# albertz/ParseOggVorbis

Measured on AMD Instinct MI355X. Metric: audio packets/sec (blocksize 2048, stereo), higher is better.
Workload: dtype f32; 1 GPU; config3: 65536 stereo packets, blocksize 2048, 64 streams x 1024, floor+coupling+IMDCT+window+overlap-add; packets_per_gpu=65536, parallelism=streams sharded over 1 GPU(s), no data-path collective

## Files before the change

parseoggvorbis_amd/csrc/vorbis_synth_hip.hip:

```cpp
#include <hip/hip_runtime.h>

#include <mutex>
#include <string>

#include <stdlib.h>

#include "vsyn_host.h"
#include "vsyn_device.h"
#include "vsyn_staged.h"
#include "vsyn_prep.h"
#include "vsyn_fused.h"
#include "vsyn_fused_u.h"
#include "vsyn_vq.h"
#include "vsyn_pcm.h"
#include "vsyn_features.h"
#include "vsyn_spectral.h"
#include "vsyn_spectral_lin.h"
#include "vsyn_spectral_post.h"
#include "vsyn_resample.h"
#include "vsyn_condition.h"
#include "vsyn_trim.h"
#include "vsyn_split.h"
#include "vsyn_pitch.h"
#include "vsyn_fdesc.h"
// ... 349 lines not shown
      fail(err, VSYN_ERR_HIP, "generic fused table upload failed: %s", hipGetErrorString(e));
      return cleanup(VSYN_ERR_HIP);
    }
  }
#undef HC
  *out = h;
  return VSYN_OK;
}

void vsyn_destroy(vsyn_handle* h) {
  if (!h) return;
  (void)hipSetDevice(h->device);
  (void)hipDeviceSynchronize();
  vq_stamps_dump();
  prep_stamps_dump();
  fused_stamps_dump();
  fused_tables_destroy(&h->fused);
  u_tables_destroy(&h->utab);
  if (h->side) (void)hipStreamDestroy(h->side);
  if (h->pre) (void)hipStreamDestroy(h->pre);
  if (h->host_stream) (void)hipStreamDestroy(h->host_stream);
  if (h->ev_join) (void)hipEventDestroy(h->ev_join);
  if (h->ev_self) (void)hipEventDestroy(h->ev_self);
  if (h->ev_reset) (void)hipEventDestroy(h->ev_reset);
  for (uint32_t b = 0; b < vsyn_handle::WS_RING; ++b)
    if (h->ev_pre_done[b]) (void)hipEventDestroy(h->ev_pre_done[b]);
  for (uint32_t b = 0; b < vsyn_handle::EV_RING; ++b)
    if (h->ev_ring[b]) (void)hipEventDestroy(h->ev_ring[b]);
  if (h->d_const) (void)hipFree(h->d_const);
  if (h->d_vq) (void)hipFree(h->d_vq);
  if (h->d_state) (void)hipFree(h->d_state);
  if (h->d_carry) (void)hipFree(h->d_carry);
  if (h->d_status) (void)hipFree(h->d_status);
  for (auto& ev : h->events) {
    (void)hipEventDestroy(ev.first);
    (void)hipEventDestroy(ev.second);
  }
  delete h;
}

uint32_t vsyn_ys_stride(const vsyn_handle* h) { return h ? h->H.ys_stride : 0; }
uint32_t vsyn_channels(const vsyn_handle* h) { return h ? h->H.channels : 0; }
uint32_t vsyn_fused_paths(const vsyn_handle* h) { return h ? (h->fused_mask | (h->vq_tables_in_lds ? 0x100u : 0u)) : 0; }
size_t vsyn_const_block_bytes(const vsyn_handle* h) { return h ? h->host_const.size() : 0; }

int vsyn_profile_enable(vsyn_handle* h, int on) {
  if (!h) return VSYN_ERR_INVALID;
  h->profile = on != 0;
  if (on >= 1 && on <= 3) h->profile_which = on;
  return VSYN_OK;
}

int vsyn_profile_read(vsyn_handle* h, double* mean_ms, uint32_t* launches, const char** kernel_name) {
  if (!h) return VSYN_ERR_INVALID;
  std::lock_guard<std::mutex> lk(h->mu);
  (void)hipSetDevice(h->device);
  double total = 0;
  for (size_t i = 0; i < h->events_used; ++i) {
    (void)hipEventSynchronize(h->events[i].second);
    float ms = 0;
    (void)hipEventElapsedTime(&ms, h->events[i].first, h->events[i].second);
    total += ms;
  }
  if (mean_ms) *mean_ms = h->events_used ? total / (double)h->events_used : 0.0;
  if (launches) *launches = (uint32_t)h->events_used;
  if (kernel_name) *kernel_name = h->profile_kernel;
  h->events_used = 0;
  return VSYN_OK;
}

static hipError_t profile_begin(vsyn_handle* h, hipStream_t s, const char* name) {
  if (!h->profile) return hipSuccess;
  if (h->events_used == h->events.size()) {
    hipEvent_t a, b;
    const unsigned pf = hipEventDisableSystemFence;
    hipError_t e = hipEventCreateWithFlags(&a, pf);
    if (e != hipSuccess) return e;
    e = hipEventCreateWithFlags(&b, pf);
    if (e != hipSuccess) return e;
    h->events.emplace_back(a, b);
  }
  h->profile_kernel = name;
  return hipEventRecord(h->events[h->events_used].first, s);
}
static hipError_t profile_end(vsyn_handle* h, hipStream_t s) {
  if (!h->profile) return hipSuccess;
  hipError_t e = hipEventRecord(h->events[h->events_used].second, s);
  ++h->events_used;
  return e;
}

int vsyn_reset_streams(vsyn_handle* h, void* hip_stream, const char** err) {
  if (!h) return fail(err, VSYN_ERR_INVALID, "handle is NULL");
  std::lock_guard<std::mutex> lk(h->mu);
  HIPCHK(hipSetDevice(h->device));
  HIPCHK(hipMemsetAsync(h->d_state, 0, sizeof(StreamState) * 2 * h->H.max_streams, (hipStream_t)hip_stream));
  HIPCHK(hipEventRecord(h->ev_reset, (hipStream_t)hip_stream));
  h->reset_pending = true;
  return VSYN_OK;
}

int vsyn_sync_status(vsyn_handle* h, void* hip_stream, vsyn_status* status, const char** err) {
  if (!h) return fail(err, VSYN_ERR_INVALID, "handle is NULL");
  HIPCHK(hipSetDevice(h->device));
  HIPCHK(hipStreamSynchronize((hipStream_t)hip_stream));
  DevStatus ds;
  HIPCHK(hipMemcpy(&ds, h->d_status, sizeof(ds), hipMemcpyDeviceToHost));
  if (ds.flags) {
    DevStatus init = {0u, 0xFFFFFFFFu};
    HIPCHK(hipMemcpy(h->d_status, &init, sizeof(init), hipMemcpyHostToDevice));
  }
  if (status) {
    status->flags = ds.flags;
    status->first_bad_packet = ds.first_bad_packet;
  }
  if (ds.flags) return fail(err, VSYN_ERR_STREAM, "device flagged the batch: flags=0x%x first_bad_packet=%u", ds.flags, ds.first_bad_packet);
  return VSYN_OK;
}

static int submit_device_impl(vsyn_handle* h, uint32_t P, const vsyn_packet* d_packets, uint32_t S, const vsyn_segment* d_segments,
                              uint32_t max_seg_packets, const uint16_t* d_ys, const vsyn_vq_batch* d_vq, float* d_residue, float* d_pcm,
                              uint64_t plane_stride, uint32_t* d_emit_len, const vsyn_taps* taps, uint32_t flags, void* hip_stream,
                              const char** err) {
  if (!h) return fail(err, VSYN_ERR_INVALID, "handle is NULL");
  if (P == 0 || S == 0) return VSYN_OK;
  if (!d_packets || !d_segments || !d_ys || !d_residue || !d_pcm) return fail(err, VSYN_ERR_INVALID, "NULL batch pointer");
  if (d_vq) {
    if (!h->d_vq) return fail(err, VSYN_ERR_INVALID, "vsyn_attach_vq has not been called on this handle");
    if (!d_vq->packets || (d_vq->num_cls && !d_vq->cls) || (d_vq->num_entries && !d_vq->entries)) return fail(err, VSYN_ERR_INVALID, "NULL vq batch pointer");
  }
  if (max_seg_packets == 0 || max_seg_packets > P) max_seg_packets = P;
  std::lock_guard<std::mutex> lk(h->mu);
  HIPCHK(hipSetDevice(h->device));
  hipStream_t s = (hipStream_t)hip_stream;
  const ConstHeader& H = h->H;
  const uint32_t C = H.channels;

  const bool want_taps = taps && (taps->after_envelope || taps->pcm_after_mdct);
  const bool use_u = h->u_mixed;
  const uint32_t fmask = h->fused_mask;
  const bool force_staged = want_taps || (flags & VSYN_SUBMIT_STAGED) || !fmask;
  const uint32_t R = force_staged ? std::min<uint32_t>(max_seg_packets, 1024u)
                                  : fused_pick_run_len(h->opt.run_len, (fmask & 1u) || !use_u ? h->fused.waves_per_cu : (int)h->utab.waves_per_cu,
                                                       S, C, max_seg_packets, h->num_cus);
  const uint32_t runs_per_seg = (max_seg_packets + R - 1) / R;

  const bool prep_kernel = !force_staged && (fmask & 2u) && !d_vq && max_seg_packets <= PREP_MAX_SEG_PACKETS && !(flags & VSYN_SUBMIT_PRE_KERNELS);
  hipStream_t ps = !prep_kernel && (flags & VSYN_SUBMIT_INPUTS_READY) && !force_staged ? h->pre : s;
  const uint32_t chunk_packets = max_seg_packets <= LAYOUT_CHUNK_PACKETS ? runs_per_seg * R : (LAYOUT_CHUNK_PACKETS + R - 1u) / R * R;
  const uint32_t chunks_per_seg = (max_seg_packets + chunk_packets - 1u) / chunk_packets;
  const uint32_t prep_nt = std::min<uint32_t>(PREP_THREADS, std::max<uint32_t>(64u, ((max_seg_packets * C + 63u) / 64u) * 64u));
  const uint32_t prep_chunk_runs = std::max<uint32_t>(1u, std::max<uint32_t>(1u, prep_nt / C) / R);
  const uint32_t prep_chunks_per_seg = (runs_per_seg + prep_chunk_runs - 1u) / prep_chunk_runs;
  const uint64_t prep_wgs = (((uint64_t)S * prep_chunks_per_seg + 7u) / 8u) * 16u;
  const bool staged_may_work = force_staged || !(fmask & 2u);
  hipStream_t ss = force_staged ? s : h->side;
  const uint64_t fused_units = (uint64_t)S * runs_per_seg * C;

  if (!prep_kernel && (uint64_t)S * chunks_per_seg > 0x7FFFFFFFull) return fail(err, VSYN_ERR_INVALID, "too many layout chunks");
  if (prep_kernel && prep_wgs > 0x7FFFFFF0ull) return fail(err, VSYN_ERR_INVALID, "too many runs");
  if (!force_staged && fused_units > (use_u ? U_MAX_UNITS : FUSED_MAX_UNITS)) return fail(err, VSYN_ERR_INVALID, "too many runs");
  const uint64_t isub = h->nsub;
  const uint32_t wb = (uint32_t)(isub % vsyn_handle::WS_RING), wb_prev = (uint32_t)((isub + vsyn_handle::WS_RING - 1u) % vsyn_handle::WS_RING);
  HIPCHK(h->ws_info[wb].ensure((size_t)P + 8));
  HIPCHK(h->ws_seg[wb].ensure(S));
  HIPCHK(h->ws_segmap[wb].ensure(P));
  HIPCHK(h->ws_list[wb].ensure(2 * (size_t)P + 64));
  uint16_t* fy = taps && taps->floor_final ? taps->floor_final : nullptr;
  if (!fy) {
    HIPCHK(h->ws_fy[wb].ensure((size_t)P * C * H.ys_stride));
    fy = h->ws_fy[wb].p;
  }
  HIPCHK(h->ws_runcls[wb].ensure((size_t)S * runs_per_seg + 16));
  bool clear_chunks = false;
  if (!prep_kernel && chunks_per_seg > 1 && (size_t)S * chunks_per_seg > h->ws_chunks.cap) {
    HIPCHK(h->ws_chunks.ensure((size_t)S * chunks_per_seg));
    clear_chunks = true;
  }
  float* env = taps && taps->after_envelope ? taps->after_envelope : nullptr;
  float* blk = taps && taps->pcm_after_mdct ? taps->pcm_after_mdct : nullptr;
  if (staged_may_work) {
    const size_t bound = (size_t)P * C * (H.bs[1] / 2);
    if (!env) {
      HIPCHK(h->ws_env.ensure(bound));
      env = h->ws_env.p;
    }
    if (!blk) {
      HIPCHK(h->ws_blk.ensure(2 * bound));
      blk = h->ws_blk.p;
    }
  }
  PktInfo* info = h->ws_info[wb].p;
  SegInfo* sinfo = h->ws_seg[wb].p;
  uint32_t* segmap = h->ws_segmap[wb].p;
  uint32_t* list = h->ws_list[wb].p;

  ++h->nsub;
  uint32_t* cnt = h->ws_count.p + (isub % vsyn_handle::CNT_RING);
  uint32_t* cnt_next = h->ws_count.p + ((isub + 1u) % vsyn_handle::CNT_RING);
  ++h->submit_count;
  const uint32_t epoch = (h->submit_count & 0x3FFFFFFFu) ? h->submit_count : ++h->submit_count;
  if (ps != s) {
    if (isub >= vsyn_handle::WS_RING) {
      const uint64_t need = isub - vsyn_handle::WS_RING;
      const uint32_t slot = (uint32_t)(need % vsyn_handle::EV_RING);
      if (h->ev_ring_submit[slot] == need) {
        HIPCHK(hipStreamWaitEvent(ps, h->ev_ring[slot], 0));
      } else {
        HIPCHK(hipEventRecord(h->ev_self, s));
        HIPCHK(hipStreamWaitEvent(ps, h->ev_self, 0));
      }
    }
    if (h->last_prep_on_main && isub > 0) {
      HIPCHK(hipEventRecord(h->ev_self, s));
      HIPCHK(hipStreamWaitEvent(ps, h->ev_self, 0));
    }
  }
  if (h->pre_done_valid[wb_prev] && h->last_pre_stream != ps) HIPCHK(hipStreamWaitEvent(ps, h->ev_pre_done[wb_prev], 0));
  if (h->reset_pending) HIPCHK(hipStreamWaitEvent(ps, h->ev_reset, 0));

  if (!prep_kernel) {
    if (!h->last_ran_layout) HIPCHK(hipMemsetAsync(h->ws_count.p, 0, sizeof(uint32_t) * vsyn_handle::CNT_RING, ps));
    if (clear_chunks) HIPCHK(hipMemsetAsync(h->ws_chunks.p, 0, h->ws_chunks.cap * sizeof(LayoutChunk), ps));
    const uint32_t lt = std::min(chunk_packets, max_seg_packets) <= LAYOUT_SHORT_PACKETS ? LAYOUT_THREADS_SHORT : LAYOUT_THREADS;
    vsyn_layout_kernel<<<S * chunks_per_seg, lt, layout_lds_bytes(lt, chunk_packets), ps>>>(
        h->d_const, P, d_packets, S, d_segments, plane_stride, info, sinfo, h->d_state, d_emit_len, h->d_status, R, force_staged ? 0u : fmask, list, cnt,
        cnt_next, segmap, h->ws_runcls[wb].p, runs_per_seg, chunk_packets, chunks_per_seg, h->ws_chunks.p, epoch);
    const uint32_t rows = P * C;
    vsyn_floor_unwrap_kernel<<<(rows + UNWRAP_THREADS - 1) / UNWRAP_THREADS, UNWRAP_THREADS, h->unwrap_lds_bytes, ps>>>(h->d_const, P, info, d_ys, fy,
                                                                                                                          h->d_status);
    if (d_vq) {
      if (h->profile_which == 3) HIPCHK(profile_begin(h, ps, "vsyn_residue_vq_kernel"));
      if (h->vq_tables_in_lds)
        vsyn_residue_vq_kernel<true><<<std::min<uint32_t>((P + h->vq_waves - 1u) / h->vq_waves, h->vq_grid), VQ_THREADS * h->vq_waves, h->vq_lds_bytes, ps>>>(
            h->d_const, h->d_vq, P, info, d_vq->packets, d_vq->cls, d_vq->num_cls, d_vq->entries, d_vq->num_entries, d_residue, h->d_status);
      else
        vsyn_residue_vq_kernel<false><<<std::min<uint32_t>(P, h->vq_grid), VQ_THREADS, h->vq_lds_bytes, ps>>>(
            h->d_const, h->d_vq, P, info, d_vq->packets, d_vq->cls, d_vq->num_cls, d_vq->entries, d_vq->num_entries, d_residue, h->d_status);
      if (h->profile_which == 3) HIPCHK(profile_end(h, ps));
    }
  } else {
    PrepCtx pc;
    pc.cb = h->d_const;
    pc.packets = d_packets;
    pc.segs = d_segments;
    pc.ys = d_ys;
    pc.fy = fy;
    pc.info = info;
    pc.sinfo = sinfo;
    pc.state = h->d_state;
    pc.status = h->d_status;
    pc.emit_len = d_emit_len;
    pc.run_cls = h->ws_runcls[wb].p;
    pc.plane_stride = plane_stride;
    pc.long_modes = h->long_modes;
    pc.S = S;
    pc.R = R;
    pc.runs_per_seg = runs_per_seg;
    pc.fused_ok = fmask;
    pc.P = P;
    pc.epoch = epoch;
    pc.chunk_runs = prep_chunk_runs;
    pc.chunks_per_seg = prep_chunks_per_seg;
    vsyn_prep_kernel<<<(uint32_t)prep_wgs, prep_nt, h->prep_lds_bytes, ps>>>(pc);
  }
  if (ps != s) {
    HIPCHK(hipEventRecord(h->ev_pre_done[wb], ps));
    HIPCHK(hipStreamWaitEvent(s, h->ev_pre_done[wb], 0));
  }

  if (staged_may_work) {
    if (!force_staged) {
      if (ps != s) {
        HIPCHK(hipStreamWaitEvent(h->side, h->ev_pre_done[wb], 0));
      } else {
        HIPCHK(hipEventRecord(h->ev_self, s));
        HIPCHK(hipStreamWaitEvent(h->side, h->ev_self, 0));
      }
    }
    const uint32_t grid = force_staged ? std::min<uint32_t>(P * C, 256u * 32u) : 512u;
    vsyn_spectrum_kernel<<<std::min<uint32_t>(grid, P), 256, 0, ss>>>(h->d_const, list, cnt, info, d_residue, fy, env,
                                                                      taps ? taps->floor_curve : nullptr, h->d_status);
    if (force_staged) HIPCHK(profile_begin(h, s, "vsyn_imdct_staged_kernel"));
    vsyn_imdct_staged_kernel<<<grid, 256, (size_t)H.bs[1] * 4, ss>>>(h->d_const, list, cnt, info, env, blk);
    if (force_staged) HIPCHK(profile_end(h, s));
    vsyn_overlap_kernel<<<grid, 256, 0, ss>>>(h->d_const, list, cnt, info, d_segments, sinfo, segmap, blk, d_pcm, plane_stride, h->d_carry);
  }
  if (!force_staged) {
    FusedArgs a;
    a.cb = h->d_const;
    a.binseg = h->fused.d_binseg;
    a.lds_image = h->fused.d_lds;
    a.packets = d_packets;
    a.segs = d_segments;
    a.info = info;
    a.sinfo = sinfo;
    a.run_cls = h->ws_runcls[wb].p;
    a.runs_per_seg = runs_per_seg;
    a.residue = d_residue;
    a.curve = taps ? taps->floor_curve : nullptr;
    a.fy = fy;
    a.pcm = d_pcm;
    a.carry = h->d_carry;
    a.status = h->d_status;
    a.plane_stride = plane_stride;
    a.S = S;
    a.R = R;
    a.fused_ok = use_u ? (fmask & 1u) : fmask;
    a.coupling_mode = (uint32_t)h->fused.coupling_mode;
    if (staged_may_work) HIPCHK(hipEventRecord(h->ev_join, h->side));
    const bool time_u = use_u && (h->profile_which == 2 || !(fmask & 1u));
    hipError_t e = hipSuccess;
    if (a.fused_ok) {
      if (!time_u && (h->profile_which == 1 || h->profile_which == 2)) HIPCHK(profile_begin(h, s, a.curve ? "vsyn_fused_tap_kernel" : fused_kernel_name(H)));
      e = fused_launch(H, h->fused, a, s);
      if (e != hipSuccess) return fail(err, VSYN_ERR_HIP, "fused launch failed: %s", hipGetErrorString(e));
      if (!time_u && (h->profile_which == 1 || h->profile_which == 2)) HIPCHK(profile_end(h, s));
    }
    if (use_u) {
      FusedArgs au = a;
      au.fused_ok = fmask;
      if (time_u && (h->profile_which == 1 || h->profile_which == 2)) HIPCHK(profile_begin(h, s, au.curve ? "vsyn_fused_u_tap_kernel" : "vsyn_fused_u_kernel"));
      e = u_launch(H, h->utab, au, s);
      if (e != hipSuccess) return fail(err, VSYN_ERR_HIP, "generic fused launch failed: %s", hipGetErrorString(e));
      if (time_u && (h->profile_which == 1 || h->profile_which == 2)) HIPCHK(profile_end(h, s));
    }
    if (staged_may_work) HIPCHK(hipStreamWaitEvent(s, h->ev_join, 0));
  }

  h->last_ran_layout = !prep_kernel;
  h->last_prep_on_main = ps == s;
  h->pre_done_valid[wb] = ps != s;
  h->last_pre_stream = ps;
  h->reset_pending = false;
  if (ps != s) {
    const uint32_t slot = (uint32_t)(isub % vsyn_handle::EV_RING);
    HIPCHK(hipEventRecord(h->ev_ring[slot], s));
    h->ev_ring_submit[slot] = isub;
  }
  h->last_S = S;
  h->last_wb = wb;
  HIPCHK(hipGetLastError());
  return VSYN_OK;
}

int vsyn_submit_device(vsyn_handle* h, uint32_t P, const vsyn_packet* d_packets, uint32_t S, const vsyn_segment* d_segments,
                       uint32_t max_seg_packets, const uint16_t* d_ys, const float* d_residue, float* d_pcm,
                       uint64_t plane_stride, uint32_t* d_emit_len, const vsyn_taps* taps, uint32_t flags, void* hip_stream,
                       const char** err) {
  return submit_device_impl(h, P, d_packets, S, d_segments, max_seg_packets, d_ys, nullptr, const_cast<float*>(d_residue), d_pcm, plane_stride,
                            d_emit_len, taps, flags, hip_stream, err);
}

int vsyn_submit_device_vq(vsyn_handle* h, uint32_t P, const vsyn_packet* d_packets, uint32_t S, const vsyn_segment* d_segments,
                          uint32_t max_seg_packets, const uint16_t* d_ys, const vsyn_vq_batch* d_vq, float* d_residue, float* d_pcm,
                          uint64_t plane_stride, uint32_t* d_emit_len, const vsyn_taps* taps, uint32_t flags, void* hip_stream,
                          const char** err) {
  if (!d_vq) return fail(err, VSYN_ERR_INVALID, "vq batch is NULL");
  return submit_device_impl(h, P, d_packets, S, d_segments, max_seg_packets, d_ys, d_vq, d_residue, d_pcm, plane_stride, d_emit_len, taps, flags,
                            hip_stream, err);
}

int vsyn_attach_vq(vsyn_handle* h, const vsyn_vq_setup* vq, const char** err) {
  if (!h) return fail(err, VSYN_ERR_INVALID, "handle is NULL");
  std::vector<uint8_t> block;
  const std::string why = vq_build_block(vq, h->H, block);
  if (!why.empty()) return fail(err, VSYN_ERR_INVALID, "%s", why.c_str());
  std::lock_guard<std::mutex> lk(h->mu);
  HIPCHK(hipSetDevice(h->device));
  const uint32_t lds_budget = 156u * 1024u;
  HIPCHK(hipFuncSetAttribute((const void*)vsyn_residue_vq_kernel<true>, hipFuncAttributeMaxDynamicSharedMemorySize, (int)lds_budget));
  HIPCHK(hipDeviceSynchronize());
  if (h->d_vq) (void)hipFree(h->d_vq);
  h->d_vq = nullptr;
  HIPCHK(hipMalloc((void**)&h->d_vq, block.size()));
  HIPCHK(hipMemcpy(h->d_vq, block.data(), block.size(), hipMemcpyHostToDevice));
  const VqHeader* vh = (const VqHeader*)block.data();
  uint32_t lds_off[7];
  const uint32_t wave_bytes = vq_lds_layout(vh->max_slots, vh->max_classes, lds_off);
  h->vq_tables_in_lds = false;
  h->vq_waves = 1;
  if (vh->img_floats && !h->opt.vq_no_lds_tables) {
    const uint32_t tab_bytes = vq_align16(vh->img_floats * 4u);
    hipFuncAttributes fa;
    HIPCHK(hipFuncGetAttributes(&fa, (const void*)vsyn_residue_vq_kernel<true>));
    const uint32_t regs = ((uint32_t)std::max(fa.numRegs, 1) + 7u) / 8u * 8u;
    const uint32_t cu_waves = 4u * std::min<uint32_t>(8u, 512u / regs);
    uint32_t best_k = 0, best_w = 0;
    for (uint32_t k = 1; k <= 4; ++k) {
      const uint32_t budget = k == 1 ? lds_budget : 128u * 1024u;
      if (budget / k <= tab_bytes + wave_bytes) break;
      const uint32_t w = std::min<uint32_t>({16u, (budget / k - tab_bytes) / wave_bytes, cu_waves / k});
      if (w && k * w > best_k * best_w) best_k = k, best_w = w;
    }
    if (best_w) {
      const uint32_t lds = tab_bytes + best_w * wave_bytes;
      int per_cu = 0;
      HIPCHK(hipOccupancyMaxActiveBlocksPerMultiprocessor(&per_cu, vsyn_residue_vq_kernel<true>, (int)(VQ_THREADS * best_w), lds));
      if (per_cu > 0) {
        h->vq_tables_in_lds = true;
        h->vq_waves = best_w;
        h->vq_lds_bytes = lds;
        h->vq_grid = (uint32_t)h->num_cus * (uint32_t)per_cu;
        if (h->opt.debug) fprintf(stderr, "[vsyn] vq: tables in LDS (%u B), %u waves per workgroup, %d workgroups per CU, %u B LDS\n", tab_bytes, best_w, per_cu, lds);
      }
    }
  }
  if (!h->vq_tables_in_lds) {
    h->vq_lds_bytes = wave_bytes;
    int per_cu = 0;
    HIPCHK(hipOccupancyMaxActiveBlocksPerMultiprocessor(&per_cu, vsyn_residue_vq_kernel<false>, VQ_THREADS, h->vq_lds_bytes));
    h->vq_grid = (uint32_t)h->num_cus * (uint32_t)std::max(per_cu, 1);
  }
  return VSYN_OK;
}

// ... 1105 lines not shown
```

parseoggvorbis_amd/csrc/vsyn_prep.h:

```cpp
#pragma once
#include <hip/hip_runtime.h>

#include "vsyn_device.h"
#include "vsyn_floor1.h"
#include "vsyn_staged.h"

#define PREP_MAX_SEG_PACKETS 4096u
#define PREP_WAVES 4
#define PREP_THREADS (PREP_WAVES * 64)

struct PrepCtx {
  const uint8_t* cb;
  const vsyn_packet* packets;
  const vsyn_segment* segs;
  const uint16_t* ys;
  uint16_t* fy;
  PktInfo* info;
  SegInfo* sinfo;
  StreamState* state;
  DevStatus* status;
  uint32_t* emit_len;
  uint8_t* run_cls;
  uint64_t plane_stride, long_modes;
  uint32_t S, R, runs_per_seg, fused_ok, P, epoch;
  uint32_t chunk_runs, chunks_per_seg;
};

#ifdef PREP_STAMPS
#define PREP_NSTAMPS 8
__device__ unsigned long long g_prep_stamps[8192][PREP_NSTAMPS];
#define PSTAMP(i)                                                \
  do {                                                           \
    __builtin_amdgcn_sched_barrier(0);                           \
    const unsigned long long t_ = __builtin_readcyclecounter();  \
    pst_acc[i] += t_ - pst_last;                                 \
    pst_last = t_;                                               \
    __builtin_amdgcn_sched_barrier(0);                           \
  } while (0)
#else
#define PSTAMP(i) do { } while (0)
#endif

__device__ __forceinline__ void prep_wave_scan(AbsScan& inc, uint64_t& rinc, const uint32_t lane) {
#pragma unroll
  for (int d = 1; d < 64; d <<= 1) {
    const AbsScan o = abs_shfl_up(inc, d);
    const uint64_t ro = __shfl_up(rinc, d);
    if ((int)lane >= d) {
      inc = abs_combine(o, inc);
      rinc += ro;
    }
  }
}
__device__ __forceinline__ uint64_t prep_readlane64(uint64_t v, uint32_t l) {
  return (uint64_t)(uint32_t)__builtin_amdgcn_readlane((uint32_t)v, l) | ((uint64_t)(uint32_t)__builtin_amdgcn_readlane((uint32_t)(v >> 32), l) << 32);
}

__device__ __forceinline__ void prep_block_scan(AbsScan& inc, uint64_t& rinc, AbsScan* s_abs, uint64_t* s_res, AbsScan* total, uint64_t* rtotal) {
  const uint32_t lane = threadIdx.x & 63u, wv = threadIdx.x >> 6;
  prep_wave_scan(inc, rinc, lane);
  __syncthreads();
  if (lane == 63u) {
    s_abs[wv] = inc;
    s_res[wv] = rinc;
  }
  __syncthreads();
  AbsScan pre = {0, 0}, tot = {0, 0};
  uint64_t rpre = 0, rtot = 0;
  const uint32_t nw = blockDim.x >> 6;
#pragma unroll
  for (uint32_t w = 0; w < PREP_WAVES; ++w) {
    if (w >= nw) break;
    const AbsScan a = s_abs[w];
    const uint64_t r = s_res[w];
    if (w < wv) {
      pre = abs_combine(pre, a);
      rpre += r;
    }
    tot = abs_combine(tot, a);
    rtot += r;
  }
  inc = abs_combine(pre, inc);
  rinc += rpre;
  *total = tot;
  *rtotal = rtot;
}

__global__ void __launch_bounds__(PREP_THREADS) vsyn_prep_kernel(const PrepCtx A) {
  extern __shared__ __attribute__((aligned(16))) uint32_t s_rows[];
  __shared__ AbsScan s_abs[PREP_WAVES];
  __shared__ uint64_t s_res[PREP_WAVES];
  __shared__ uint32_t s_pk[PREP_THREADS];
  __shared__ uint32_t s_longbits[PREP_MAX_SEG_PACKETS / 32 + 2];
  __shared__ uint32_t s_last_n;
  const uint8_t* __restrict__ cb = A.cb;
  const ConstHeader* H = hdr_of(cb);
  const uint32_t t = threadIdx.x, lane = t & 63u, wave = __builtin_amdgcn_readfirstlane(t >> 6);
  const uint32_t NT = blockDim.x;
  const uint32_t C = H->channels;
  const uint32_t xj = blockIdx.x >> 3;
  const uint32_t role = (xj ^ (xj >> 5)) & 1u, bid = ((xj >> 1) << 3) | (blockIdx.x & 7u);
  const uint32_t g = bid / A.chunks_per_seg, ch = bid % A.chunks_per_seg;
  if (g >= A.S) return;
#ifdef PREP_STAMPS
  unsigned long long pst_acc[PREP_NSTAMPS] = {0, 0, 0, 0, 0, 0, 0, 0};
  unsigned long long pst_last = __builtin_readcyclecounter();
  const unsigned long long pst_t0 = __builtin_amdgcn_s_memrealtime();
#define PSTAMP_FLUSH()                                                                                              \
  do {                                                                                                              \
    const uint32_t unit_ = blockIdx.x * PREP_WAVES + wave;                                                          \
    if (lane == 0 && unit_ < 8192) {                                                                                \
      for (int i_ = 0; i_ < 5; ++i_) g_prep_stamps[unit_][i_] = pst_acc[i_];                                        \
      g_prep_stamps[unit_][5] = pst_t0;                                                                             \
      g_prep_stamps[unit_][6] = __builtin_amdgcn_s_memrealtime();                                                   \
      g_prep_stamps[unit_][7] = 1ull + role;                                                                        \
    }                                                                                                               \
  } while (0)
#else
#define PSTAMP_FLUSH() do { } while (0)
#endif
  const vsyn_segment sg = A.segs[g];
  const uint32_t num = sg.num_packets;
  const uint32_t R = A.R;
  const uint32_t run0 = ch * A.chunk_runs;
  const uint32_t run1 = min(A.runs_per_seg, run0 + A.chunk_runs);
  const uint32_t cs = run0 * R;
  uint8_t* const cls_row = A.run_cls + (size_t)g * A.runs_per_seg;
  if (sg.stream >= H->max_streams || (uint64_t)sg.first_packet + sg.num_packets > A.P || (sg.residue_off & 3)) {
    if (role) return;
    for (uint32_t r = run0 + t; r < run1; r += NT) cls_row[r] = 0xFFu;
    if (ch == 0u && t == 0u) {
      raise_status(A.status, VSYN_ST_BAD_SEGMENT, sg.first_packet < A.P ? sg.first_packet : 0);
      A.sinfo[g] = SegInfo{0, 0, 0, 0};
    }
    return;
  }
  const uint32_t ce = min(num, run1 * R);
  const vsyn_packet* const spk = A.packets + sg.first_packet;
  typedef uint32_t u32x4 __attribute__((ext_vector_type(4)));
  const uint32_t num_modes = H->num_modes, bs0 = H->bs[0], bs1 = H->bs[1];
  const uint64_t long_modes = A.long_modes;
#define PREP_IS_LONG(m) ((m) < num_modes && (m) < 64u && ((long_modes >> (m)) & 1ull))
#define PREP_N_OF_MODE(m) (PREP_IS_LONG(m) ? bs1 : bs0)
  if (role) {
    const uint32_t ce = min(num, run1 * R);
    if (cs >= ce) return;
    const vsyn_packet* const spk = A.packets + sg.first_packet;
    const uint32_t stride = __builtin_amdgcn_readfirstlane(H->ys_stride);
    const MapConst* const maps = (const MapConst*)(cb + H->off_map);
    const uint32_t chan_mask = C >= 32 ? 0xFFFFFFFFu : ((1u << C) - 1u);
    const uint32_t num_modes = H->num_modes;
    const uint32_t ppp = NT / C;
    for (uint32_t base = cs; base < ce; base += ppp) {
      const uint32_t pe = min(ce, base + ppp);
      const uint32_t rp = t / C, c = t - rp * C;
      const bool row_ok = rp < pe - base;
      uint32_t kmode = 0xFFFFFFFFu, fused_mask = 0;
      if (row_ok) {
        typedef uint32_t u32x2 __attribute__((ext_vector_type(2)));
        const u32x2 w = *(const u32x2*)(spk + base + rp);
        kmode = w.x & 0xFFu;
        fused_mask = w.y;
      }
      const bool mode_ok = row_ok && kmode < num_modes;
      uint32_t fl_id = 0xFFFFFFFFu;
      {
        typedef const __attribute__((address_space(4))) uint32_t* kptr;
        uint64_t todo = __ballot(mode_ok);
        while (todo) {
          const uint32_t m = __builtin_amdgcn_readlane(kmode, (uint32_t)__builtin_ctzll(todo));
          const bool mine = mode_ok && kmode == m;
          todo &= ~__ballot(mine);
          const uint32_t mw = *(kptr)(uintptr_t)((const uint8_t*)H->mode_mapping + (m & ~3u));
          const uint32_t mp = (mw >> (8u * (m & 3u))) & 0xFFu;
          if (mine) fl_id = maps[mp].chfloor[c];
        }
      }
      const bool act = mode_ok && (((fused_mask & chan_mask) >> c) & 1u);
      const uint32_t prow = sg.first_packet + base + rp;
      PSTAMP(3);
      floor1_unwrap_rows(A.cb, A.ys, A.fy, A.status, act, fl_id, prow, (size_t)prow * C + c, stride, (floor1_lds_u32*)s_rows + t, NT);
      PSTAMP(4);
    }
    PSTAMP_FLUSH();
    return;
  }
  uint32_t st_slot;
  const StreamState st0 = state_read(A.state, sg.stream, A.epoch, &st_slot);
  const bool reset = (sg.flags & VSYN_SEG_RESET) != 0;
  const uint32_t carry_n = (!reset && st0.has_prev) ? st0.prev_n : 0;
  const int64_t abs0 = reset ? 0 : (int64_t)st0.abs_total_pos;
  SegInfo si;
  si.has_carry = carry_n ? 1u : 0u;
  si.carry_n = carry_n;
  si.parity_in = reset ? 0u : st0.parity;
  si.total_emit = 0;
  if (cs >= num) {
    for (uint32_t r = run0 + t; r < run1; r += NT) cls_row[r] = 0xFFu;
    if (num == 0u && ch == 0u && t == 0u) {
      A.sinfo[g] = si;
      if (reset) state_write(A.state, sg.stream, st_slot, StreamState{0, 0, 0, 0, 0}, A.epoch);
    }
    return;
  }
  PSTAMP(0);

  AbsScan cin = {0, 0};
  uint64_t cres = 0;
  uint32_t prev_n_in = carry_n;
  uint32_t prev_tail_in = carry_n ? st0.prev_tail : 0u;
  bool halo_long = !carry_n;
  if (cs > 0u) {
    const uint32_t per = (cs + NT - 1u) / NT;
    const uint32_t b = min(cs, t * per), e = min(cs, b + per);
    AbsScan agg = {0, 0};
    uint64_t res = 0;
    uint32_t prev_n = 0;
    if (b < e) prev_n = b == 0u ? carry_n : PREP_N_OF_MODE((uint32_t)spk[b - 1u].mode);
    constexpr uint32_t KEEP = 8;
    for (uint32_t base = b; base < e; base += KEEP) {
      u32x4 kq[KEEP];
#pragma unroll
      for (uint32_t j = 0; j < KEEP; ++j)
        if (base + j < e) kq[j] = *(const u32x4*)(spk + base + j);
#pragma unroll
      for (uint32_t j = 0; j < KEEP; ++j)
        if (base + j < e) {
          const uint32_t md = kq[j].x & 0xFFu;
          const uint32_t n = PREP_N_OF_MODE(md);
          const int64_t gran = (int64_t)((uint64_t)kq[j].z | ((uint64_t)kq[j].w << 32));
          agg = abs_combine(agg, abs_element(gran, prev_n ? (int64_t)(prev_n / 4 + n / 4) : 0));
          res += (uint64_t)C * (n / 2);
          prev_n = n;
        }
    }
    prep_block_scan(agg, res, s_abs, s_res, &cin, &cres);
    const uint32_t hm = __builtin_amdgcn_readfirstlane((uint32_t)spk[cs - 1u].mode);
    prev_n_in = PREP_N_OF_MODE(hm);
    halo_long = PREP_IS_LONG(hm);
    prev_tail_in = prev_tail_of(PREP_IS_LONG(hm), (uint8_t)__builtin_amdgcn_readfirstlane((uint32_t)spk[cs - 1u].next_long));
  }
  PSTAMP(1);

  const uint32_t stride = __builtin_amdgcn_readfirstlane(H->ys_stride);
  const MapConst* const maps = (const MapConst*)(cb + H->off_map);
  const uint32_t chan_mask = C >= 32 ? 0xFFFFFFFFu : ((1u << C) - 1u);
  const uint32_t ppp = NT / C;
  for (uint32_t w = t; w < (ce - cs + 1u + 31u) / 32u; w += NT) s_longbits[w] = 0u;
  __syncthreads();
  if (t == 0u && halo_long) s_longbits[0] = 1u;
  for (uint32_t base = cs; base < ce; base += ppp) {
    const uint32_t pe = min(ce, base + ppp);
    const uint32_t q = base + t;
    const bool valid = q < pe;
    vsyn_packet k = {};
    if (valid) {
      const u32x4 w = *(const u32x4*)(spk + q);
      k.mode = (uint8_t)(w.x & 0xFFu);
      k.prev_long = (uint8_t)((w.x >> 8) & 0xFFu);
      k.next_long = (uint8_t)((w.x >> 16) & 0xFFu);
      k.floor_used = w.y;
      k.granule = (int64_t)((uint64_t)w.z | ((uint64_t)w.w << 32));
    }
    const bool mode_ok = valid && k.mode < num_modes;
    const uint32_t kmode = k.mode;
    const uint32_t lng = (valid && PREP_IS_LONG(kmode)) ? 1u : 0u;
    const uint32_t n = lng ? bs1 : bs0;
    __syncthreads();
    const uint32_t tail = prev_tail_of(mode_ok && lng, k.next_long);
    s_pk[t] = n | (tail << 31);
    __syncthreads();
    const uint32_t prev_n = t == 0u ? prev_n_in : (s_pk[t - 1u] & 0x7FFFFFFFu);
    const uint32_t prev_tail = t == 0u ? prev_tail_in : (s_pk[t - 1u] >> 31);
    AbsScan inc = {0, 0};
    uint64_t rinc = 0;
    if (valid) {
      inc = abs_element(k.granule, prev_n ? (int64_t)(prev_n / 4 + n / 4) : 0);
      rinc = (uint64_t)C * (n / 2);
    }
    const AbsScan own_el = inc;
    const uint64_t own_res = rinc;
    AbsScan tot;
    uint64_t rtot;
    prep_block_scan(inc, rinc, s_abs, s_res, &tot, &rtot);
    const uint64_t rex = rinc - own_res;
    AbsScan ex;
    {
      ex = abs_shfl_up(inc, 1);
      if (lane == 0u) {
        AbsScan pre = {0, 0};
        for (uint32_t w = 0; w < wave; ++w) pre = abs_combine(pre, s_abs[w]);
        ex = pre;
      }
    }
    (void)own_el;
    ex = abs_combine(cin, ex);
    const int64_t abs_before = abs_eval(ex, abs0);
    const uint64_t res_off = sg.residue_off + cres + rex;
    const uint32_t p = sg.first_packet + q;
    uint32_t mapping = 0, own = k.floor_used & chan_mask, used = own;
    {
      typedef const __attribute__((address_space(4))) uint32_t* kptr;
      uint64_t todo = __ballot(mode_ok);
      while (todo) {
        const uint32_t m = __builtin_amdgcn_readlane(kmode, (uint32_t)__builtin_ctzll(todo));
        const bool mine = mode_ok && kmode == m;
        todo &= ~__ballot(mine);
        const uint32_t mw = *(kptr)(uintptr_t)((const uint8_t*)H->mode_mapping + (m & ~3u));
        const uint32_t mp = (mw >> (8u * (m & 3u))) & 0xFFu;
        const MapConst* mc = maps + mp;
        const uint32_t ncoup = *(kptr)(uintptr_t)&mc->ncoup;
        uint32_t u = used;
        for (uint32_t i = 0; i < ncoup; ++i) {
          const uint32_t pair = *(kptr)(uintptr_t)&mc->coup[2 * i];
          const uint32_t ma = pair & 0xFFFFu, an = pair >> 16;
          if (((u >> ma) | (u >> an)) & 1u) u |= (1u << ma) | (1u << an);
        }
        if (mine) {
          mapping = mp;
          used = u;
        }
      }
    }
    if (valid) {
      const PktStep ps = pkt_step_core(k, mode_ok, lng, mapping, n, prev_n, prev_tail, abs_before, abs0, res_off, A.plane_stride, own, used);
      if (ps.raise) {
        if (ps.raise & VSYN_ST_BAD_MODE) raise_status(A.status, VSYN_ST_BAD_MODE, p);
        if (ps.raise & VSYN_ST_WINDOW_FLAGS) raise_status(A.status, VSYN_ST_WINDOW_FLAGS, p);
        if (ps.raise & VSYN_ST_GRANULE) raise_status(A.status, VSYN_ST_GRANULE, p);
        if (ps.raise & VSYN_ST_PLANE_OVERFLOW) raise_status(A.status, VSYN_ST_PLANE_OVERFLOW, p);
      }
      A.info[p] = ps.pi;
      if (A.emit_len) A.emit_len[p] = ps.pi.emit;
      if (q == num - 1u) {
        SegInfo so = si;
        so.total_emit = (uint32_t)(ps.abs_after - abs0);
        A.sinfo[g] = so;
        StreamState ns;
        ns.abs_total_pos = (uint64_t)ps.abs_after;
        ns.has_prev = 1;
        ns.prev_n = n;
        ns.prev_tail = tail;
        ns.parity = si.parity_in ^ 1u;
        ns.tag = 0;
        state_write(A.state, sg.stream, st_slot, ns, A.epoch);
      }
      if (mode_ok && lng) atomicOr(&s_longbits[(q - cs + 1u) >> 5], 1u << ((q - cs + 1u) & 31u));
      if (q == pe - 1u) s_last_n = n | (tail << 31);
    }
    __syncthreads();
    PSTAMP(2);
    cin = abs_combine(cin, tot);
    cres += rtot;
    prev_n_in = s_last_n & 0x7FFFFFFFu;
    prev_tail_in = s_last_n >> 31;
  }
  __syncthreads();
  {
    const uint32_t nruns_seg = (num + R - 1u) / R;
    for (uint32_t r = run0 + t; r < run1; r += NT) {
      uint32_t cls = 0xFFu;
      if (r < nruns_seg) {
        const uint32_t first = r * R - cs, end = min(num, (r + 1u) * R) - cs;
        bool all_long = true;
        for (uint32_t w = first >> 5; all_long && w <= (end >> 5); ++w) {
          uint32_t need = 0xFFFFFFFFu;
          if (w == (first >> 5)) need &= 0xFFFFFFFFu << (first & 31u);
          if (w == (end >> 5)) need &= 0xFFFFFFFFu >> (31u - (end & 31u));
          all_long = (s_longbits[w] & need) == need;
        }
        cls = (all_long && (A.fused_ok & 1u)) ? 1u : ((A.fused_ok & 2u) ? 2u : 0u);
      }
      cls_row[r] = (uint8_t)cls;
    }
  }
  PSTAMP_FLUSH();
#undef PREP_IS_LONG
#undef PREP_N_OF_MODE
}

#include <stdio.h>

static inline void prep_stamps_dump() {
#ifdef PREP_STAMPS
  static unsigned long long host[8192][PREP_NSTAMPS];
  if (hipMemcpyFromSymbol(host, HIP_SYMBOL(g_prep_stamps), sizeof(host)) == hipSuccess) {
    unsigned long long t_first = ~0ull;
    for (int u = 0; u < 8192; ++u)
      if (host[u][7] && host[u][5] < t_first) t_first = host[u][5];
    for (unsigned role = 0; role < 2; ++role) {
      double sum[5] = {0}, st = 0, en = 0, en_max = 0, st_max = 0;
      unsigned long long waves = 0;
      for (int u = 0; u < 8192; ++u) {
        if (host[u][7] != 1ull + role) continue;
        ++waves;
        for (int i = 0; i < 5; ++i) sum[i] += (double)host[u][i];
        const double a = (double)(host[u][5] - t_first) / 100.0, b = (double)(host[u][6] - t_first) / 100.0;
        st += a;
        en += b;
        if (a > st_max) st_max = a;
        if (b > en_max) en_max = b;
      }
      if (!waves) continue;
      static const char* nm[5] = {"header + stream state", "scan in front of the chunk", "descriptors, scan, PktInfo", "floor role: descriptors, floor ids", "floor role: chains"};
      fprintf(stderr, "prep stamps, %s role: %llu waves; start %.2f us (latest %.2f), end %.2f us (latest %.2f) after the launch's first wave\n",
              role ? "floor" : "layout", waves, st / waves, st_max, en / waves, en_max);
      for (int i = 0; i < 5; ++i)
        if (sum[i] > 0) fprintf(stderr, "  %-36s %8.0f cycles\n", nm[i], sum[i] / waves);
    }
  }
#endif
}
```

Measured before the change: 272.5 million packets/s.

## Split prep kernel roles by grid range and replace LDS neighbor exchange with shuffles

The prep kernel now splits its grid into a contiguous range of layout workgroups, whose chunk size is tied to the thread count, followed by the other role's workgroups. This replaces the old interleaved XOR-based role mapping. The previous-packet values (n, tail) are now obtained with a wave shuffle plus a direct global load of the neighbouring packet word for lane 0. That removes the shared s_pk array, s_last_n and two block barriers per iteration. Packet words are prefetched one iteration ahead to hide load latency. The risks are that the cross-wave and cross-iteration carries now depend on PREP_N_OF_MODE and re-reading packets, and that the grid size and role balance change.

```diff
diff --git a/parseoggvorbis_amd/csrc/vorbis_synth_hip.hip b/parseoggvorbis_amd/csrc/vorbis_synth_hip.hip
--- a/parseoggvorbis_amd/csrc/vorbis_synth_hip.hip
+++ b/parseoggvorbis_amd/csrc/vorbis_synth_hip.hip
@@ -525,7 +525,10 @@
   const uint32_t prep_nt = std::min<uint32_t>(PREP_THREADS, std::max<uint32_t>(64u, ((max_seg_packets * C + 63u) / 64u) * 64u));
   const uint32_t prep_chunk_runs = std::max<uint32_t>(1u, std::max<uint32_t>(1u, prep_nt / C) / R);
   const uint32_t prep_chunks_per_seg = (runs_per_seg + prep_chunk_runs - 1u) / prep_chunk_runs;
-  const uint64_t prep_wgs = (((uint64_t)S * prep_chunks_per_seg + 7u) / 8u) * 16u;
+  const uint32_t prep_lchunk_runs = std::max<uint32_t>(1u, PREP_LAYOUT_PACKETS / R);
+  const uint32_t prep_lchunks_per_seg = (runs_per_seg + prep_lchunk_runs - 1u) / prep_lchunk_runs;
+  const uint64_t prep_layout_wgs = (uint64_t)S * prep_lchunks_per_seg;
+  const uint64_t prep_wgs = prep_layout_wgs + (uint64_t)S * prep_chunks_per_seg;
   const bool staged_may_work = force_staged || !(fmask & 2u);
   hipStream_t ss = force_staged ? s : h->side;
   const uint64_t fused_units = (uint64_t)S * runs_per_seg * C;
@@ -635,6 +638,9 @@
     pc.epoch = epoch;
     pc.chunk_runs = prep_chunk_runs;
     pc.chunks_per_seg = prep_chunks_per_seg;
+    pc.lchunk_runs = prep_lchunk_runs;
+    pc.lchunks_per_seg = prep_lchunks_per_seg;
+    pc.n_layout = (uint32_t)prep_layout_wgs;
     vsyn_prep_kernel<<<(uint32_t)prep_wgs, prep_nt, h->prep_lds_bytes, ps>>>(pc);
   }
   if (ps != s) {
diff --git a/parseoggvorbis_amd/csrc/vsyn_prep.h b/parseoggvorbis_amd/csrc/vsyn_prep.h
--- a/parseoggvorbis_amd/csrc/vsyn_prep.h
+++ b/parseoggvorbis_amd/csrc/vsyn_prep.h
@@ -8,6 +8,7 @@
 #define PREP_MAX_SEG_PACKETS 4096u
 #define PREP_WAVES 4
 #define PREP_THREADS (PREP_WAVES * 64)
+#define PREP_LAYOUT_PACKETS PREP_THREADS
 
 struct PrepCtx {
   const uint8_t* cb;
@@ -24,6 +25,8 @@
   uint64_t plane_stride, long_modes;
   uint32_t S, R, runs_per_seg, fused_ok, P, epoch;
   uint32_t chunk_runs, chunks_per_seg;
+  uint32_t lchunk_runs, lchunks_per_seg;
+  uint32_t n_layout;
 };
 
 #ifdef PREP_STAMPS
@@ -90,17 +93,16 @@
   extern __shared__ __attribute__((aligned(16))) uint32_t s_rows[];
   __shared__ AbsScan s_abs[PREP_WAVES];
   __shared__ uint64_t s_res[PREP_WAVES];
-  __shared__ uint32_t s_pk[PREP_THREADS];
   __shared__ uint32_t s_longbits[PREP_MAX_SEG_PACKETS / 32 + 2];
-  __shared__ uint32_t s_last_n;
   const uint8_t* __restrict__ cb = A.cb;
   const ConstHeader* H = hdr_of(cb);
   const uint32_t t = threadIdx.x, lane = t & 63u, wave = __builtin_amdgcn_readfirstlane(t >> 6);
   const uint32_t NT = blockDim.x;
   const uint32_t C = H->channels;
-  const uint32_t xj = blockIdx.x >> 3;
-  const uint32_t role = (xj ^ (xj >> 5)) & 1u, bid = ((xj >> 1) << 3) | (blockIdx.x & 7u);
-  const uint32_t g = bid / A.chunks_per_seg, ch = bid % A.chunks_per_seg;
+  const uint32_t role = blockIdx.x >= A.n_layout ? 1u : 0u;
+  const uint32_t bid = role ? blockIdx.x - A.n_layout : blockIdx.x;
+  const uint32_t cps = role ? A.chunks_per_seg : A.lchunks_per_seg, cruns = role ? A.chunk_runs : A.lchunk_runs;
+  const uint32_t g = bid / cps, ch = bid % cps;
   if (g >= A.S) return;
 #ifdef PREP_STAMPS
   unsigned long long pst_acc[PREP_NSTAMPS] = {0, 0, 0, 0, 0, 0, 0, 0};
@@ -122,8 +124,8 @@
   const vsyn_segment sg = A.segs[g];
   const uint32_t num = sg.num_packets;
   const uint32_t R = A.R;
-  const uint32_t run0 = ch * A.chunk_runs;
-  const uint32_t run1 = min(A.runs_per_seg, run0 + A.chunk_runs);
+  const uint32_t run0 = ch * cruns;
+  const uint32_t run1 = min(A.runs_per_seg, run0 + cruns);
   const uint32_t cs = run0 * R;
   uint8_t* const cls_row = A.run_cls + (size_t)g * A.runs_per_seg;
   if (sg.stream >= H->max_streams || (uint64_t)sg.first_packet + sg.num_packets > A.P || (sg.residue_off & 3)) {
@@ -245,17 +247,28 @@
   const uint32_t stride = __builtin_amdgcn_readfirstlane(H->ys_stride);
   const MapConst* const maps = (const MapConst*)(cb + H->off_map);
   const uint32_t chan_mask = C >= 32 ? 0xFFFFFFFFu : ((1u << C) - 1u);
-  const uint32_t ppp = NT / C;
+  const uint32_t ppp = NT;
   for (uint32_t w = t; w < (ce - cs + 1u + 31u) / 32u; w += NT) s_longbits[w] = 0u;
   __syncthreads();
   if (t == 0u && halo_long) s_longbits[0] = 1u;
+  u32x4 w_next = {0u, 0u, 0u, 0u};
+  uint32_t wp_next = 0u;
+  if (cs + t < ce) {
+    w_next = *(const u32x4*)(spk + cs + t);
+    if (lane == 0u && t > 0u) wp_next = *(const uint32_t*)(spk + cs + t - 1u);
+  }
   for (uint32_t base = cs; base < ce; base += ppp) {
     const uint32_t pe = min(ce, base + ppp);
     const uint32_t q = base + t;
     const bool valid = q < pe;
     vsyn_packet k = {};
+    const u32x4 w = w_next;
+    const uint32_t wp = wp_next;
+    if (base + ppp + t < ce) {
+      w_next = *(const u32x4*)(spk + base + ppp + t);
+      if (lane == 0u) wp_next = *(const uint32_t*)(spk + base + ppp + t - 1u);
+    }
     if (valid) {
-      const u32x4 w = *(const u32x4*)(spk + q);
       k.mode = (uint8_t)(w.x & 0xFFu);
       k.prev_long = (uint8_t)((w.x >> 8) & 0xFFu);
       k.next_long = (uint8_t)((w.x >> 16) & 0xFFu);
@@ -266,12 +279,14 @@
     const uint32_t kmode = k.mode;
     const uint32_t lng = (valid && PREP_IS_LONG(kmode)) ? 1u : 0u;
     const uint32_t n = lng ? bs1 : bs0;
-    __syncthreads();
     const uint32_t tail = prev_tail_of(mode_ok && lng, k.next_long);
-    s_pk[t] = n | (tail << 31);
-    __syncthreads();
-    const uint32_t prev_n = t == 0u ? prev_n_in : (s_pk[t - 1u] & 0x7FFFFFFFu);
-    const uint32_t prev_tail = t == 0u ? prev_tail_in : (s_pk[t - 1u] >> 31);
+    uint32_t prev_pk = __shfl_up(n | (tail << 31), 1);
+    if (lane == 0u) {
+      const uint32_t pm = wp & 0xFFu;
+      prev_pk = q == cs ? (prev_n_in | (prev_tail_in << 31)) : (PREP_N_OF_MODE(pm) | (prev_tail_of(PREP_IS_LONG(pm), (uint8_t)((wp >> 16) & 0xFFu)) << 31));
+    }
+    const uint32_t prev_n = prev_pk & 0x7FFFFFFFu;
+    const uint32_t prev_tail = prev_pk >> 31;
     AbsScan inc = {0, 0};
     uint64_t rinc = 0;
     if (valid) {
@@ -346,14 +361,10 @@
         state_write(A.state, sg.stream, st_slot, ns, A.epoch);
       }
       if (mode_ok && lng) atomicOr(&s_longbits[(q - cs + 1u) >> 5], 1u << ((q - cs + 1u) & 31u));
-      if (q == pe - 1u) s_last_n = n | (tail << 31);
-    }
-    __syncthreads();
+    }
     PSTAMP(2);
     cin = abs_combine(cin, tot);
     cres += rtot;
-    prev_n_in = s_last_n & 0x7FFFFFFFu;
-    prev_tail_in = s_last_n >> 31;
   }
   __syncthreads();
   {
```

Result: no change. 275.4 million packets/s, median of 3 (+1.1%).
